# OpenDriveLab/Vista

Hardware: NVIDIA H100
Metric: denoised frames/sec at 25x576x1024, 50 EDM steps; UNet step ms (higher is better)
Workload: dtype f16 (fp32 accumulate, fp32 norms/softmax/sampler state)

## Files before the change

### vista_b200/csrc/gemm_tc.cu

```cuda
#include "gemm_tc.cuh"

namespace vb {
extern template const GemmKern* gemm_variants<32>();
extern template const GemmKern* gemm_variants<64>();
extern template const GemmKern* gemm_variants<96>();
extern template const GemmKern* gemm_variants<128>();
extern template const GemmKern* gemm_variants<160>();
extern template const GemmKern* gemm_variants<192>();
extern template const GemmKern* gemm_variants<224>();
extern template const GemmKern* gemm_variants<256>();
}

extern "C" int b200v_gemm(const b200v_gemm_desc* d, void* stream_) {
  using namespace vb;
  cudaStream_t stream = reinterpret_cast<cudaStream_t>(stream_);
  VB_REQUIRE(d && d->a && d->b && d->out, "b200v_gemm: null pointer");
  VB_REQUIRE(d->cin > 0 && d->cin % 64 == 0, "b200v_gemm: cin=%d must be a positive multiple of 64", d->cin);
  VB_REQUIRE(d->ntaps >= 1 && d->ntaps <= 9, "b200v_gemm: ntaps=%d out of range", d->ntaps);
  VB_REQUIRE(d->N > 0 && d->N % 8 == 0, "b200v_gemm: N=%d must be a multiple of 8", d->N);
  VB_REQUIRE(d->tile_n >= 32 && d->tile_n <= 256 && d->tile_n % 32 == 0, "b200v_gemm: tile_n=%d invalid", d->tile_n);
  VB_REQUIRE(d->lda % 8 == 0 && d->ldo % 8 == 0, "b200v_gemm: lda/ldo must be multiples of 8");
  VB_REQUIRE(d->act >= 0 && d->act <= 3, "b200v_gemm: act=%d invalid", d->act);
  VB_REQUIRE(!(d->act == 2 && (d->tile_n % 64 != 0 || d->N % d->tile_n != 0 || d->out_f32)),
             "b200v_gemm: GEGLU needs tile_n %% 64 == 0, N %% tile_n == 0, 16-bit output");
  VB_REQUIRE(!(d->act == 2 && (d->rowvec || d->res1 || d->res2)), "b200v_gemm: GEGLU epilogue takes bias only");
  VB_REQUIRE(!(d->act == 3 && (d->rowvec || d->res1 || d->res2 || d->bf16 || d->out_f32 || d->stats)),
             "b200v_gemm: the GELU epilogue takes bias only, fp16 operands and output (compiled variant)");
  VB_REQUIRE(!d->res1 || d->ld_res1 % 8 == 0, "b200v_gemm: ld_res1 must be a multiple of 8");
  VB_REQUIRE(!d->res2 || d->ld_res2 % 8 == 0, "b200v_gemm: ld_res2 must be a multiple of 8");
  VB_REQUIRE(!d->rowvec || (d->ld_rowvec % 4 == 0 && d->rv_div > 0 && d->rv_mod > 0), "b200v_gemm: bad rowvec args");
  VB_REQUIRE((reinterpret_cast<uintptr_t>(d->a) & 15) == 0 && (reinterpret_cast<uintptr_t>(d->b) & 15) == 0 &&
                 (reinterpret_cast<uintptr_t>(d->out) & 15) == 0,
             "b200v_gemm: a/b/out must be 16-byte aligned");

  TGParams p;
  memset(&p, 0, sizeof(p));
  p.a_mode = d->a_mode;
  p.tokens = d->tokens;
  const long long K = (long long)d->ntaps * d->cin;
  CUtensorMap tmA, tmB;
  if (d->a_mode == 0) {
    VB_REQUIRE(d->ntaps == 1 && d->h_pad == 0, "b200v_gemm: linear mode takes one tap and no halo rows");
    VB_REQUIRE(d->tokens > 0 && d->tokens < (1ll << 31) - 256, "b200v_gemm: tokens out of range");
    p.W = (int)d->tokens; p.H = 1; p.NB = 1;
    p.BW = 128; p.BH = 1; p.BB = 1;
    p.tiles_w = (int)((d->tokens + 127) / 128); p.tiles_h = 1;
    p.m_tiles = p.tiles_w;
    uint64_t dims[2] = {(uint64_t)d->cin, (uint64_t)d->tokens};
    uint64_t strides[1] = {(uint64_t)d->lda * 2};
    uint32_t box[2] = {64, 128};
    uint32_t es[2] = {1, 1};
    if (encode_tmap_16bit(&tmA, d->a, 2, dims, strides, box, es, d->bf16)) return 3;
  } else {
    VB_REQUIRE(d->a_mode == 1 || d->a_mode == 2, "b200v_gemm: a_mode=%d invalid", d->a_mode);
    const long long out_tokens = d->a_mode == 2 ? 4ll * d->tokens : d->tokens;
    VB_REQUIRE(d->W > 0 && d->H > 0 && d->NB > 0 && (long long)d->W * d->H * d->NB == d->tokens &&
                   out_tokens < (1ll << 31) - 256,
               "b200v_gemm: W*H*NB != tokens (or output tokens >= 2^31)");
    VB_REQUIRE(d->a_mode == 1 || (d->h_pad == 0 && d->act == 0 && !d->rowvec && !d->res1 && !d->res2 && !d->bf16 &&
                                  !d->out_f32 && d->s_acc == 1.0f),
               "b200v_gemm: the upsampling mode (a_mode 2) takes bias and fused statistics only, fp16 in and out");
    VB_REQUIRE(d->box_w > 0 && d->box_h > 0 && d->box_b > 0 && d->box_w * d->box_h * d->box_b == 128,
               "b200v_gemm: box_w*box_h*box_b must be 128");
    p.W = d->W; p.H = d->H; p.NB = d->NB;
    p.BW = d->box_w; p.BH = d->box_h; p.BB = d->box_b;
    p.tiles_w = (d->W + p.BW - 1) / p.BW;
    p.tiles_h = (d->H + p.BH - 1) / p.BH;
    const int tiles_b = (d->NB + p.BB - 1) / p.BB;
    p.m_tiles = p.tiles_w * p.tiles_h * tiles_b * (d->a_mode == 2 ? 4 : 1);
    VB_REQUIRE(d->h_pad >= 0 && d->h_pad <= 4, "b200v_gemm: h_pad=%d out of range", d->h_pad);
    const uint64_t He = (uint64_t)d->H + 2ull * d->h_pad;
    uint64_t dims[4] = {(uint64_t)d->cin, (uint64_t)d->W, He, (uint64_t)d->NB};
    uint64_t strides[3] = {(uint64_t)d->lda * 2, (uint64_t)d->lda * 2 * d->W, (uint64_t)d->lda * 2 * d->W * He};
    uint32_t box[4] = {64, (uint32_t)p.BW, (uint32_t)p.BH, (uint32_t)p.BB};
    uint32_t es[4] = {1, 1, 1, 1};
    if (encode_tmap_16bit(&tmA, d->a, 4, dims, strides, box, es, d->bf16)) return 3;
  }
  {
    uint64_t dims[2] = {(uint64_t)K, (uint64_t)d->N};
    uint64_t strides[1] = {(uint64_t)K * 2};
    uint32_t box[2] = {64, (uint32_t)d->tile_n};
    uint32_t es[2] = {1, 1};
    if (encode_tmap_16bit(&tmB, d->b, 2, dims, strides, box, es, d->bf16)) return 3;
  }
  p.ntaps = d->ntaps;
  p.kc_per_tap = d->cin / 64;
  for (int i = 0; i < 9; ++i) {
    p.dh[i] = d->dh[i] + (d->a_mode == 1 ? d->h_pad : 0);
    p.dw[i] = d->dw[i];
  }
  p.N = d->N;
  p.n_tiles = (d->N + d->tile_n - 1) / d->tile_n;
  p.stage_bytes = kABytes + ((d->tile_n * 128 + 1023) / 1024) * 1024;
  constexpr int kMaxSmem = 227 * 1024;
  p.nstages = (kMaxSmem - 2048 - kStagingBytes) / p.stage_bytes;
  if (p.nstages > kMaxStages) p.nstages = kMaxStages;
  const long long kMaxLd = (1ll << 31) - 1;
  VB_REQUIRE(d->ldo * (d->out_f32 ? 4 : 2) <= kMaxLd && d->ld_rowvec * 4 <= kMaxLd && d->ld_res1 * 2 <= kMaxLd &&
                 d->ld_res2 * 2 <= kMaxLd,
             "b200v_gemm: row stride too large");
  for (p.bw_sh = 0; (1 << p.bw_sh) < p.BW; ++p.bw_sh) {}
  for (p.bh_sh = 0; (1 << p.bh_sh) < p.BH; ++p.bh_sh) {}
  p.out = d->out; p.ldo_b = (int)(d->ldo * (d->out_f32 ? 4 : 2)); p.out_f32 = d->out_f32; p.act = d->act;
  p.bias = d->bias;
  p.rowvec = d->rowvec; p.ld_rowvec_b = (int)(d->ld_rowvec * 4); p.rv_div = d->rv_div > 0 ? d->rv_div : 1;
  p.rv_mod = d->rv_mod > 0 ? d->rv_mod : 1;
  p.res1 = d->res1; p.ld_res1_b = (int)(d->ld_res1 * 2); p.s_res1 = d->s_res1;
  p.res2 = d->res2; p.ld_res2_b = (int)(d->ld_res2 * 2); p.s_res2 = d->s_res2;
  p.s_acc = d->s_acc;
  VB_REQUIRE(!(d->res2 && !d->res1), "b200v_gemm: res2 without res1");
  p.stats = d->stats; p.stats_ld = (int)d->stats_ld; p.stats_col0 = d->stats_col0;
  if (d->stats) {
    VB_REQUIRE(!d->bf16 && !d->out_f32 && d->act == 0 && !d->res2 && !(d->rowvec && d->res1),
               "b200v_gemm: fused statistics need fp16 output, act 0, <= 1 residual and no rowvec + residual");
    VB_REQUIRE(d->stats_ld >= d->stats_col0 + d->N && d->stats_col0 % 4 == 0 && d->stats_ld % 4 == 0 &&
                   (reinterpret_cast<uintptr_t>(d->stats) & 15) == 0,
               "b200v_gemm: bad stats_ld / stats_col0 / alignment");
    VB_REQUIRE(d->a_mode == 0 || (p.BB == 1 && d->W % p.BW == 0 && d->H % p.BH == 0 &&
                                  (d->a_mode == 2 || p.BW == d->W || p.BH == 1)),
               "b200v_gemm: fused statistics need token tiles of 128 consecutive tokens, or boxes that tile each frame "
               "in upsampling mode (box %d x %d x %d on %d x %d)",
               p.BW, p.BH, p.BB, d->W, d->H);
  }

  const int smem_bytes = 1024 + 1024 + p.nstages * p.stage_bytes + kStagingBytes;
  int variant = d->bf16 ? 12 : 7;
  if (d->stats) {
    variant = 9 + (d->rowvec ? 2 : (d->res1 ? 1 : 0));
  } else if (!d->bf16 && !d->out_f32) {
    const int nres = (d->res1 ? 1 : 0) + (d->res2 ? 1 : 0);
    if (d->act == 0 && !d->rowvec) variant = nres;
    else if (d->act == 0 && nres <= 1) variant = 3 + nres;
    else if (d->act == 1 && !d->rowvec && nres == 0) variant = 5;
    else if (d->act == 2) variant = 6;
    else if (d->act == 3) variant = 8;
  }
  static const GemmKern* const kByWidth[8] = {gemm_variants<32>(),  gemm_variants<64>(),  gemm_variants<96>(),
                                              gemm_variants<128>(), gemm_variants<160>(), gemm_variants<192>(),
                                              gemm_variants<224>(), gemm_variants<256>()};
  static bool attr_set[64] = {false};
  if (vb::first_use_on_device(attr_set)) {
    for (int w = 0; w < 8; ++w)
      for (int i = 0; i < kGemmVariants; ++i)
        VB_CHECK_CUDA(cudaFuncSetAttribute(kByWidth[w][i], cudaFuncAttributeMaxDynamicSharedMemorySize, kMaxSmem));
  }
  const long long total = (long long)p.m_tiles * p.n_tiles;
  int grid = device_sm_count();
  if (total < grid) grid = (int)total;
  const GemmKern k = kByWidth[d->tile_n / 32 - 1][variant];
  k<<<grid, kGemmThreads, smem_bytes, stream>>>(tmA, tmB, p);
  VB_CHECK_CUDA(cudaGetLastError());
  return 0;
}
```

### vista_b200/csrc/gemm_tc.cuh

```cuda
#pragma once
#include "../../include/vista_b200.h"
#include "host.cuh"
#include "ptx.cuh"

namespace vb {

constexpr int kMaxStages = 8;
constexpr int kABytes = 128 * 64 * 2;
constexpr int kStageBufBytes = 64 * 32 * 4;
constexpr int kStagingBytes = 2 * 2 * kStageBufBytes;
constexpr int kGemmThreads = 384;

struct TGParams {
  int a_mode;
  int W, H, NB;
  int BW, BH, BB;
  int bw_sh, bh_sh;
  int tiles_w, tiles_h;
  int m_tiles, n_tiles;
  int ntaps, kc_per_tap;
  int dh[9], dw[9];
  int N;
  int nstages, stage_bytes;
  long long tokens;
  void* out;
  int ldo_b;
  int out_f32, act;
  const float* bias;
  const float* rowvec;
  int ld_rowvec_b;
  int rv_div, rv_mod;
  const void* res1;
  int ld_res1_b;
  float s_res1;
  const void* res2;
  int ld_res2_b;
  float s_res2;
  float s_acc;
  float* stats;
  int stats_ld, stats_col0;
};

__device__ __forceinline__ float2 unpack2(uint32_t w, int bf16) {
  if (bf16) return make_float2(__uint_as_float(w << 16), __uint_as_float(w & 0xFFFF0000u));
  return __half22float2(*reinterpret_cast<const __half2*>(&w));
}
__device__ __forceinline__ uint32_t pack2(float a, float b, int bf16) {
  if (bf16) {
    __nv_bfloat162 t = __floats2bfloat162_rn(a, b);
    return *reinterpret_cast<uint32_t*>(&t);
  }
  __half2 t = __floats2half2_rn(a, b);
  return *reinterpret_cast<uint32_t*>(&t);
}

template <int TN, bool BF16>
__device__ __forceinline__ void issue_kchunk(float (&acc)[TN / 2], uint64_t adesc, uint64_t bdesc, bool overwrite) {
#pragma unroll
  for (int kk = 0; kk < 4; ++kk)
    wgmma_ss<TN, BF16>(acc, adesc + (uint64_t)(2 * kk), bdesc + (uint64_t)(2 * kk), (overwrite && kk == 0) ? 0 : 1);
}

template <int TN, int ACT_, bool RV_, int NRES_, bool GEN, bool STATS = false, bool BF16 = false>
__global__ void __launch_bounds__(kGemmThreads, 1)
tapgemm_kernel(const __grid_constant__ CUtensorMap tmA, const __grid_constant__ CUtensorMap tmB, const TGParams p) {
  extern __shared__ uint8_t smem_raw[];
  const uint32_t raw = smem_u32(smem_raw);
  uint8_t* smem = smem_raw + (((raw + 1023u) & ~1023u) - raw);
  uint64_t* full = reinterpret_cast<uint64_t*>(smem);
  uint64_t* empty = full + kMaxStages;
  uint8_t* stages = smem + 1024;

  const int warp = threadIdx.x >> 5, lane = threadIdx.x & 31;
  const int KC = p.ntaps * p.kc_per_tap;
  const int total_tiles = p.m_tiles * p.n_tiles;

  if (threadIdx.x == 0) {
    for (int i = 0; i < p.nstages; ++i) {
      mbar_init(&full[i], 1);
      mbar_init(&empty[i], 8);
    }
    fence_barrier_init();
  }
  if (warp == 8 && lane == 0) {
    tma_prefetch_desc(&tmA);
    tma_prefetch_desc(&tmB);
  }
  __syncthreads();

  if (warp >= 8) {
    setmaxnreg_dec<40>();
    if (warp == 8 && lane == 0) {
      int stage = 0;
      uint32_t phase = 0;
      const uint32_t tx = (uint32_t)(kABytes + TN * 128);
      for (int tile = blockIdx.x; tile < total_tiles; tile += gridDim.x) {
        const int m_blk = tile / p.n_tiles, n_blk = tile - m_blk * p.n_tiles;
        const int up = p.a_mode == 2;
        const int box = up ? (m_blk >> 2) : m_blk;
        const int px = up ? (m_blk & 1) : 0, py = up ? ((m_blk >> 1) & 1) : 0;
        const int tw = box % p.tiles_w;
        const int th = (box / p.tiles_w) % p.tiles_h;
        const int tb = box / (p.tiles_w * p.tiles_h);
        const int w0 = tw * p.BW, h0 = th * p.BH, b0 = tb * p.BB;
        const int n0 = n_blk * TN;
        for (int kc = 0; kc < KC; ++kc) {
          mbar_wait_relaxed(&empty[stage], phase ^ 1, 1);
          uint8_t* sA = stages + stage * p.stage_bytes;
          uint8_t* sB = sA + kABytes;
          const int tap = kc / p.kc_per_tap;
          const int c0 = (kc - tap * p.kc_per_tap) * 64;
          mbar_expect_tx(&full[stage], tx);
          const int dw = up ? ((px + p.dw[tap]) >> 1) : p.dw[tap];
          const int dh = up ? ((py + p.dh[tap]) >> 1) : p.dh[tap];
          if (p.a_mode == 0)
            tma_load_2d(sA, &tmA, &full[stage], c0, w0);
          else
            tma_load_4d(sA, &tmA, &full[stage], c0, w0 + dw, h0 + dh, b0);
          tma_load_2d(sB, &tmB, &full[stage], kc * 64, n0);
          if (++stage == p.nstages) {
            stage = 0;
            phase ^= 1;
          }
        }
      }
    }
    return;
  }

  setmaxnreg_inc<232>();
  const int wg = warp >> 2, wq = warp & 3;
  const int act = GEN ? p.act : ACT_;
  const bool has_rv = GEN ? (p.rowvec != nullptr) : RV_;
  const bool has_r1 = GEN ? (p.res1 != nullptr) : (NRES_ >= 1);
  const bool has_r2 = GEN ? (p.res2 != nullptr) : (NRES_ >= 2);
  constexpr bool bf16 = BF16;
  const bool f32o = GEN ? (p.out_f32 != 0) : false;
  const bool has_bias = p.bias != nullptr;
  constexpr int half = TN >> 1;
  const int tile_out_cols = (act == 2) ? half : TN;
  const int n_out_total = (act == 2) ? (p.N >> 1) : p.N;
  const int G = tile_out_cols >> 5;
  const int out_es = f32o ? 4 : 2;
  const char* r1p = reinterpret_cast<const char*>(p.res1);
  const char* r2p = reinterpret_cast<const char*>(p.res2);
  const uint64_t desc0 = make_desc_sw128(smem_u32(stages), 16, 1024);
  const uint32_t stage_step = (uint32_t)p.stage_bytes >> 4;
  const uint32_t stg0 = smem_u32(stages + p.nstages * p.stage_bytes) + wg * 2 * kStageBufBytes;
  const int g = lane >> 2, c = lane & 3;
  const int rh = wq & 1, chh = wq >> 1;
  const int ch = lane & 3, rsub = lane >> 2;
  int stage = 0;
  uint32_t phase = 0;
  uint32_t gcount = 0;

  float acc[TN / 2];
  for (int tile = blockIdx.x; tile < total_tiles; tile += gridDim.x) {
    const int m_blk = tile / p.n_tiles, n_blk = tile - m_blk * p.n_tiles;
    int prev = -1;
    for (int kc = 0; kc < KC; ++kc) {
      mbar_wait(&full[stage], phase, 3);
      const uint64_t ad = desc0 + (uint64_t)(stage * stage_step + wg * 512);
      const uint64_t bd = desc0 + (uint64_t)(stage * stage_step + (kABytes >> 4));
      wgmma_fence();
      issue_kchunk<TN, BF16>(acc, ad, bd, kc == 0);
      wgmma_commit();
      if (prev >= 0) {
        wgmma_wait<1>();
        if (lane == 0) mbar_arrive(&empty[prev]);
      }
      prev = stage;
      if (++stage == p.nstages) {
        stage = 0;
        phase ^= 1;
      }
    }
    wgmma_wait<0>();
    if (lane == 0) mbar_arrive(&empty[prev]);
    fence_regs(acc);

    const int r_own = wg * 64 + rh * 32 + lane;
    int token_own, valid_own;
    if (p.a_mode == 0) {
      token_own = m_blk * 128 + r_own;
      valid_own = token_own < p.tokens;
    } else {
      const int up = p.a_mode == 2;
      const int box = up ? (m_blk >> 2) : m_blk;
      const int tw = box % p.tiles_w;
      const int t2 = box / p.tiles_w;
      const int th = t2 % p.tiles_h;
      const int tb = t2 / p.tiles_h;
      const int ww = r_own & (p.BW - 1), hh = (r_own >> p.bw_sh) & (p.BH - 1), bb = r_own >> (p.bw_sh + p.bh_sh);
      const int w = tw * p.BW + ww, h = th * p.BH + hh, b = tb * p.BB + bb;
      valid_own = (w < p.W) && (h < p.H) && (b < p.NB);
      token_own = up ? ((2 * (b * p.H + h) + ((m_blk >> 1) & 1)) * 2 * p.W + 2 * w + (m_blk & 1))
                     : (b * p.H + h) * p.W + w;
    }
    if (!valid_own) token_own = 0;
    const uint32_t vrows = __ballot_sync(0xffffffffu, valid_own) >> rsub;
    int tok[4], rvrow[4];
    {
      const int rv_own = has_rv ? (token_own / p.rv_div) % p.rv_mod : 0;
#pragma unroll
      for (int i = 0; i < 4; ++i) {
        tok[i] = __shfl_sync(0xffffffffu, token_own, i * 8 + rsub);
        rvrow[i] = has_rv ? __shfl_sync(0xffffffffu, rv_own, i * 8 + rsub) : 0;
      }
    }
    const int n_out_base = n_blk * tile_out_cols;
#pragma unroll
    for (int k = 0; k < TN / 32; ++k) {
      if (k >= G) break;
      const int c0 = k * 32;
      if (n_out_base + c0 >= n_out_total) break;
      const uint32_t stg = stg0 + (gcount & 1) * kStageBufBytes;
      ++gcount;
      float f[16];
#pragma unroll
      for (int j = 0; j < 16; ++j) f[j] = acc[16 * k + j];
      if (act == 2) {
        float gt[16];
        const int kg = (half >> 5) + k;
#pragma unroll
        for (int j = 0; j < 16; ++j) gt[j] = 0.f;
#pragma unroll
        for (int q = 0; q < TN / 32; ++q)
          if (q == kg) {
#pragma unroll
            for (int j = 0; j < 16; ++j) gt[j] = acc[16 * q + j];
          }
        const int nb = n_blk * TN + c0;
#pragma unroll
        for (int ii = 0; ii < 4; ++ii) {
          float2 bv = make_float2(0.f, 0.f), bg = make_float2(0.f, 0.f);
          if (has_bias) {
            bv = __ldg(reinterpret_cast<const float2*>(p.bias + nb + 8 * ii + 2 * c));
            bg = __ldg(reinterpret_cast<const float2*>(p.bias + nb + half + 8 * ii + 2 * c));
          }
          f[4 * ii + 0] = geglu_fast(f[4 * ii + 0] + bv.x, gt[4 * ii + 0] + bg.x);
          f[4 * ii + 1] = geglu_fast(f[4 * ii + 1] + bv.y, gt[4 * ii + 1] + bg.y);
          f[4 * ii + 2] = geglu_fast(f[4 * ii + 2] + bv.x, gt[4 * ii + 2] + bg.x);
          f[4 * ii + 3] = geglu_fast(f[4 * ii + 3] + bv.y, gt[4 * ii + 3] + bg.y);
        }
      }
#pragma unroll
      for (int ii = 0; ii < 4; ++ii) {
        const int chunk = 2 * ii + (c >> 1), sub = (c & 1) * 8;
#pragma unroll
        for (int hr = 0; hr < 2; ++hr) {
          const int row = wq * 16 + g + 8 * hr;
          asm volatile("st.shared.v2.f32 [%0], {%1, %2};" ::"r"(stg + row * 128 + ((chunk ^ (row & 7)) << 4) + sub),
                       "f"(f[4 * ii + 2 * hr]), "f"(f[4 * ii + 2 * hr + 1])
                       : "memory");
        }
      }
      asm volatile("bar.sync %0, 128;" ::"r"(1 + wg) : "memory");
      {
        const int n = n_out_base + c0 + chh * 16 + ch * 4;
        const bool n_ok = n + 4 <= n_out_total;
        float4 bs = make_float4(0.f, 0.f, 0.f, 0.f);
        float sa = 1.0f;
        if (act != 2) {
          sa = p.s_acc;
          if (has_bias && n_ok) {
            const float4 b4 = __ldg(reinterpret_cast<const float4*>(p.bias + n));
            bs = make_float4(b4.x * sa, b4.y * sa, b4.z * sa, b4.w * sa);
          }
        }
        char* obase = reinterpret_cast<char*>(p.out) + (long long)n * out_es;
        const char* r1base = r1p + (long long)n * 2;
        const char* r2base = r2p + (long long)n * 2;
        const char* rvbase = reinterpret_cast<const char*>(p.rowvec) + (long long)n * 4;
        float cs[4] = {0.f, 0.f, 0.f, 0.f}, cq[4] = {0.f, 0.f, 0.f, 0.f};
        float4 v[4], rv[4];
        uint2 u1[4], u2[4];
#pragma unroll
        for (int i = 0; i < 4; ++i) {
          const int row = rh * 32 + i * 8 + rsub;
          const int chunk = chh * 4 + ch;
          asm volatile("ld.shared.v4.f32 {%0, %1, %2, %3}, [%4];"
                       : "=f"(v[i].x), "=f"(v[i].y), "=f"(v[i].z), "=f"(v[i].w)
                       : "r"(stg + row * 128 + ((chunk ^ (row & 7)) << 4)));
          const bool ok = n_ok && ((vrows >> (8 * i)) & 1u);
          rv[i] = make_float4(0.f, 0.f, 0.f, 0.f);
          u1[i] = make_uint2(0, 0);
          u2[i] = make_uint2(0, 0);
          if (has_rv && ok) rv[i] = __ldg(reinterpret_cast<const float4*>(rvbase + (long long)rvrow[i] * p.ld_rowvec_b));
          if (has_r1 && ok) u1[i] = __ldg(reinterpret_cast<const uint2*>(r1base + (long long)tok[i] * p.ld_res1_b));
          if (has_r2 && ok) u2[i] = __ldg(reinterpret_cast<const uint2*>(r2base + (long long)tok[i] * p.ld_res2_b));
        }
#pragma unroll
        for (int i = 0; i < 4; ++i) {
          const bool ok = n_ok && ((vrows >> (8 * i)) & 1u);
          float4 o = v[i];
          if (act != 2) {
            o.x = fmaf(o.x, sa, bs.x); o.y = fmaf(o.y, sa, bs.y); o.z = fmaf(o.z, sa, bs.z); o.w = fmaf(o.w, sa, bs.w);
            if (has_rv) { o.x += rv[i].x; o.y += rv[i].y; o.z += rv[i].z; o.w += rv[i].w; }
            if (act == 1) { o.x = silu_f(o.x); o.y = silu_f(o.y); o.z = silu_f(o.z); o.w = silu_f(o.w); }
            if (!GEN && act == 3) { o.x = gelu_erf_fast(o.x); o.y = gelu_erf_fast(o.y); o.z = gelu_erf_fast(o.z); o.w = gelu_erf_fast(o.w); }
            if (has_r1) {
              const float2 a = unpack2(u1[i].x, bf16), b = unpack2(u1[i].y, bf16);
              o.x = fmaf(p.s_res1, a.x, o.x); o.y = fmaf(p.s_res1, a.y, o.y);
              o.z = fmaf(p.s_res1, b.x, o.z); o.w = fmaf(p.s_res1, b.y, o.w);
            }
            if (has_r2) {
              const float2 a = unpack2(u2[i].x, bf16), b = unpack2(u2[i].y, bf16);
              o.x = fmaf(p.s_res2, a.x, o.x); o.y = fmaf(p.s_res2, a.y, o.y);
              o.z = fmaf(p.s_res2, b.x, o.z); o.w = fmaf(p.s_res2, b.y, o.w);
            }
          }
          if (STATS && ok) {
            cs[0] += o.x; cs[1] += o.y; cs[2] += o.z; cs[3] += o.w;
            cq[0] = fmaf(o.x, o.x, cq[0]); cq[1] = fmaf(o.y, o.y, cq[1]);
            cq[2] = fmaf(o.z, o.z, cq[2]); cq[3] = fmaf(o.w, o.w, cq[3]);
          }
          char* optr = obase + (long long)tok[i] * p.ldo_b;
          if (f32o) {
            if (ok) *reinterpret_cast<float4*>(optr) = o;
          } else {
            const uint2 pk = make_uint2(pack2(o.x, o.y, bf16), pack2(o.z, o.w, bf16));
            if (ok) *reinterpret_cast<uint2*>(optr) = pk;
          }
        }
        if (STATS) {
#pragma unroll
          for (int off = 4; off < 32; off <<= 1) {
#pragma unroll
            for (int q = 0; q < 4; ++q) {
              cs[q] += __shfl_xor_sync(0xffffffffu, cs[q], off);
              cq[q] += __shfl_xor_sync(0xffffffffu, cq[q], off);
            }
          }
          if (rsub == 0 && n_ok) {
            float* dst = p.stats + (((long long)m_blk * 4 + wg * 2 + rh) * p.stats_ld + p.stats_col0 + n) * 2;
            *reinterpret_cast<float4*>(dst) = make_float4(cs[0], cq[0], cs[1], cq[1]);
            *reinterpret_cast<float4*>(dst + 4) = make_float4(cs[2], cq[2], cs[3], cq[3]);
          }
        }
      }
    }
  }
}

using GemmKern = void (*)(const CUtensorMap, const CUtensorMap, const TGParams);
constexpr int kGemmVariants = 13;

template <int TN>
const GemmKern* gemm_variants() {
  static const GemmKern v[kGemmVariants] = {
      tapgemm_kernel<TN, 0, false, 0, false>,       tapgemm_kernel<TN, 0, false, 1, false>,
      tapgemm_kernel<TN, 0, false, 2, false>,       tapgemm_kernel<TN, 0, true, 0, false>,
      tapgemm_kernel<TN, 0, true, 1, false>,        tapgemm_kernel<TN, 1, false, 0, false>,
      tapgemm_kernel<TN, 2, false, 0, false>,       tapgemm_kernel<TN, 0, true, 2, true>,
      tapgemm_kernel<TN, 3, false, 0, false>,       tapgemm_kernel<TN, 0, false, 0, false, true>,
      tapgemm_kernel<TN, 0, false, 1, false, true>, tapgemm_kernel<TN, 0, true, 0, false, true>,
      tapgemm_kernel<TN, 0, true, 2, true, false, true>};
  return v;
}

}
```

### vista_b200/csrc/ptx.cuh

```cuda
#pragma once
#include <cuda.h>
#include <cuda_bf16.h>
#include <cuda_fp16.h>
#include <cuda_runtime.h>
#include <stdint.h>
#include <stdio.h>

namespace vb {

__device__ __forceinline__ uint32_t smem_u32(const void* p) {
  return static_cast<uint32_t>(__cvta_generic_to_shared(p));
}

__device__ __forceinline__ void mbar_init(uint64_t* bar, uint32_t count) {
  asm volatile("mbarrier.init.shared::cta.b64 [%0], %1;" ::"r"(smem_u32(bar)), "r"(count) : "memory");
}
__device__ __forceinline__ void fence_barrier_init() {
  asm volatile("fence.mbarrier_init.release.cluster;" ::: "memory");
}
__device__ __forceinline__ void mbar_expect_tx(uint64_t* bar, uint32_t bytes) {
  asm volatile("mbarrier.arrive.expect_tx.shared::cta.b64 _, [%0], %1;" ::"r"(smem_u32(bar)), "r"(bytes) : "memory");
}
__device__ __forceinline__ void mbar_arrive(uint64_t* bar) {
  asm volatile("mbarrier.arrive.shared::cta.b64 _, [%0];" ::"r"(smem_u32(bar)) : "memory");
}
__device__ __forceinline__ bool mbar_try_wait(uint64_t* bar, uint32_t parity) {
  uint32_t ok;
  asm volatile(
      "{\n\t.reg .pred p;\n\t"
      "mbarrier.try_wait.parity.shared::cta.b64 p, [%1], %2;\n\t"
      "selp.u32 %0, 1, 0, p;\n\t}"
      : "=r"(ok)
      : "r"(smem_u32(bar)), "r"(parity)
      : "memory");
  return ok != 0;
}
__device__ __forceinline__ bool mbar_test_wait(uint64_t* bar, uint32_t parity) {
  uint32_t ok;
  asm volatile(
      "{\n\t.reg .pred p;\n\t"
      "mbarrier.test_wait.parity.shared::cta.b64 p, [%1], %2;\n\t"
      "selp.u32 %0, 1, 0, p;\n\t}"
      : "=r"(ok)
      : "r"(smem_u32(bar)), "r"(parity)
      : "memory");
  return ok != 0;
}
#ifndef VB_WAIT_TIMEOUT_CYCLES
#define VB_WAIT_TIMEOUT_CYCLES (4000000000ll)
#endif
__device__ __forceinline__ void mbar_wait(uint64_t* bar, uint32_t parity, int tag = 0) {
  (void)tag;
  if (mbar_try_wait(bar, parity)) return;
  long long t0 = 0;
  for (uint32_t spins = 1;; ++spins) {
    if (mbar_try_wait(bar, parity)) return;
    if ((spins & 4095u) == 0u) {
      const long long now = clock64();
      if (t0 == 0) t0 = now;
      if (now - t0 > VB_WAIT_TIMEOUT_CYCLES) __trap();
    }
  }
}
__device__ __forceinline__ void mbar_wait_relaxed(uint64_t* bar, uint32_t parity, int tag = 0) {
  (void)tag;
  for (int i = 0; i < 4; ++i)
    if (mbar_try_wait(bar, parity)) return;
  long long t0 = 0;
  for (uint32_t spins = 1;; ++spins) {
    __nanosleep(32);
    if (mbar_try_wait(bar, parity)) return;
    if ((spins & 4095u) == 0u) {
      const long long now = clock64();
      if (t0 == 0) t0 = now;
      if (now - t0 > VB_WAIT_TIMEOUT_CYCLES) __trap();
    }
  }
}

__device__ __forceinline__ void fence_proxy_async_smem() {
  asm volatile("fence.proxy.async.shared::cta;" ::: "memory");
}

__device__ __forceinline__ void tma_prefetch_desc(const CUtensorMap* m) {
  asm volatile("prefetch.tensormap [%0];" ::"l"(reinterpret_cast<uint64_t>(m)) : "memory");
}
__device__ __forceinline__ void tma_load_2d(void* dst, const CUtensorMap* m, uint64_t* bar, int c0, int c1) {
  asm volatile(
      "cp.async.bulk.tensor.2d.shared::cluster.global.tile.mbarrier::complete_tx::bytes [%0], [%1, {%3, %4}], [%2];"
      ::"r"(smem_u32(dst)), "l"(reinterpret_cast<uint64_t>(m)), "r"(smem_u32(bar)), "r"(c0), "r"(c1)
      : "memory");
}
__device__ __forceinline__ void tma_load_3d(void* dst, const CUtensorMap* m, uint64_t* bar, int c0, int c1, int c2) {
  asm volatile(
      "cp.async.bulk.tensor.3d.shared::cluster.global.tile.mbarrier::complete_tx::bytes [%0], [%1, {%3, %4, %5}], [%2];"
      ::"r"(smem_u32(dst)), "l"(reinterpret_cast<uint64_t>(m)), "r"(smem_u32(bar)), "r"(c0), "r"(c1), "r"(c2)
      : "memory");
}
__device__ __forceinline__ void tma_load_4d(void* dst, const CUtensorMap* m, uint64_t* bar, int c0, int c1, int c2,
                                            int c3) {
  asm volatile(
      "cp.async.bulk.tensor.4d.shared::cluster.global.tile.mbarrier::complete_tx::bytes [%0], [%1, {%3, %4, %5, %6}], [%2];"
      ::"r"(smem_u32(dst)), "l"(reinterpret_cast<uint64_t>(m)), "r"(smem_u32(bar)), "r"(c0), "r"(c1), "r"(c2), "r"(c3)
      : "memory");
}

__device__ __forceinline__ uint64_t make_desc_sw128(uint32_t smem_addr, uint32_t lbo_bytes, uint32_t sbo_bytes) {
  uint64_t d = 0;
  d |= static_cast<uint64_t>((smem_addr & 0x3FFFFu) >> 4);
  d |= static_cast<uint64_t>((lbo_bytes >> 4) & 0x3FFFu) << 16;
  d |= static_cast<uint64_t>((sbo_bytes >> 4) & 0x3FFFu) << 32;
  d |= static_cast<uint64_t>(1) << 62;
  return d;
}
__device__ __forceinline__ void wgmma_fence() { asm volatile("wgmma.fence.sync.aligned;" ::: "memory"); }
__device__ __forceinline__ void wgmma_commit() { asm volatile("wgmma.commit_group.sync.aligned;" ::: "memory"); }
template <int N>
__device__ __forceinline__ void wgmma_wait() { asm volatile("wgmma.wait_group.sync.aligned %0;" ::"n"(N) : "memory"); }
template <int R>
__device__ __forceinline__ void setmaxnreg_inc() { asm volatile("setmaxnreg.inc.sync.aligned.u32 %0;" ::"n"(R)); }
template <int R>
__device__ __forceinline__ void setmaxnreg_dec() { asm volatile("setmaxnreg.dec.sync.aligned.u32 %0;" ::"n"(R)); }
template <int N>
__device__ __forceinline__ void fence_regs(float (&r)[N]) {
#pragma unroll
  for (int i = 0; i < N; ++i) asm volatile("" : "+f"(r[i])::"memory");
}

#define VB_R16_0 "%3, %4, %5, %6, %7, %8, %9, %10, %11, %12, %13, %14, %15, %16, %17, %18"
#define VB_R16_1 ", %19, %20, %21, %22, %23, %24, %25, %26, %27, %28, %29, %30, %31, %32, %33, %34"
#define VB_R16_2 ", %35, %36, %37, %38, %39, %40, %41, %42, %43, %44, %45, %46, %47, %48, %49, %50"
#define VB_R16_3 ", %51, %52, %53, %54, %55, %56, %57, %58, %59, %60, %61, %62, %63, %64, %65, %66"
#define VB_R16_4 ", %67, %68, %69, %70, %71, %72, %73, %74, %75, %76, %77, %78, %79, %80, %81, %82"
#define VB_R16_5 ", %83, %84, %85, %86, %87, %88, %89, %90, %91, %92, %93, %94, %95, %96, %97, %98"
#define VB_R16_6 ", %99, %100, %101, %102, %103, %104, %105, %106, %107, %108, %109, %110, %111, %112, %113, %114"
#define VB_R16_7 ", %115, %116, %117, %118, %119, %120, %121, %122, %123, %124, %125, %126, %127, %128, %129, %130"
#define VB_D16(b)                                                                                                      \
  "+f"(d[b + 0]), "+f"(d[b + 1]), "+f"(d[b + 2]), "+f"(d[b + 3]), "+f"(d[b + 4]), "+f"(d[b + 5]), "+f"(d[b + 6]),      \
      "+f"(d[b + 7]), "+f"(d[b + 8]), "+f"(d[b + 9]), "+f"(d[b + 10]), "+f"(d[b + 11]), "+f"(d[b + 12]),               \
      "+f"(d[b + 13]), "+f"(d[b + 14]), "+f"(d[b + 15])
#define VB_WGMMA_SS(N, T, REGS, ...)                                                                                   \
  asm volatile("{\n\t.reg .pred p;\n\tsetp.ne.b32 p, %2, 0;\n\t"                                                      \
               "wgmma.mma_async.sync.aligned.m64n" #N "k16.f32." T "." T " {" REGS "}, %0, %1, p, 1, 1, 0, 0;\n\t}" \
               : "+l"(da), "+l"(db), "+r"(scale_d), __VA_ARGS__)
#define VB_WGMMA_SS_T(N, REGS, ...)                                                                                    \
  do {                                                                                                                 \
    if constexpr (BF16) VB_WGMMA_SS(N, "bf16", REGS, __VA_ARGS__);                                                     \
    else VB_WGMMA_SS(N, "f16", REGS, __VA_ARGS__);                                                                     \
  } while (0)
template <int N, bool BF16>
__device__ __forceinline__ void wgmma_ss(float (&d)[N / 2], uint64_t da, uint64_t db, int scale_d) {
  static_assert(N >= 32 && N <= 256 && N % 32 == 0, "wgmma_ss: N must be a multiple of 32 in [32, 256]");
  if constexpr (N == 32) VB_WGMMA_SS_T(32, VB_R16_0, VB_D16(0));
  else if constexpr (N == 64) VB_WGMMA_SS_T(64, VB_R16_0 VB_R16_1, VB_D16(0), VB_D16(16));
  else if constexpr (N == 96) VB_WGMMA_SS_T(96, VB_R16_0 VB_R16_1 VB_R16_2, VB_D16(0), VB_D16(16), VB_D16(32));
  else if constexpr (N == 128)
    VB_WGMMA_SS_T(128, VB_R16_0 VB_R16_1 VB_R16_2 VB_R16_3, VB_D16(0), VB_D16(16), VB_D16(32), VB_D16(48));
  else if constexpr (N == 160)
    VB_WGMMA_SS_T(160, VB_R16_0 VB_R16_1 VB_R16_2 VB_R16_3 VB_R16_4, VB_D16(0), VB_D16(16), VB_D16(32), VB_D16(48),
                  VB_D16(64));
  else if constexpr (N == 192)
    VB_WGMMA_SS_T(192, VB_R16_0 VB_R16_1 VB_R16_2 VB_R16_3 VB_R16_4 VB_R16_5, VB_D16(0), VB_D16(16), VB_D16(32),
                  VB_D16(48), VB_D16(64), VB_D16(80));
  else if constexpr (N == 224)
    VB_WGMMA_SS_T(224, VB_R16_0 VB_R16_1 VB_R16_2 VB_R16_3 VB_R16_4 VB_R16_5 VB_R16_6, VB_D16(0), VB_D16(16),
                  VB_D16(32), VB_D16(48), VB_D16(64), VB_D16(80), VB_D16(96));
  else
    VB_WGMMA_SS_T(256, VB_R16_0 VB_R16_1 VB_R16_2 VB_R16_3 VB_R16_4 VB_R16_5 VB_R16_6 VB_R16_7, VB_D16(0), VB_D16(16),
                  VB_D16(32), VB_D16(48), VB_D16(64), VB_D16(80), VB_D16(96), VB_D16(112));
}
#undef VB_WGMMA_SS_T
#undef VB_WGMMA_SS
#undef VB_D16
#undef VB_R16_0
#undef VB_R16_1
#undef VB_R16_2
#undef VB_R16_3
#undef VB_R16_4
#undef VB_R16_5
#undef VB_R16_6
#undef VB_R16_7

__device__ __forceinline__ void wgmma_m64n128_f16(float (&d)[64], uint64_t da, uint64_t db, int scale_d) {
  asm volatile(
      "{\n\t.reg .pred p;\n\tsetp.ne.b32 p, %66, 0;\n\t"
      "wgmma.mma_async.sync.aligned.m64n128k16.f32.f16.f16 "
      "{%0, %1, %2, %3, %4, %5, %6, %7, %8, %9, %10, %11, %12, %13, %14, %15, %16, %17, %18, %19, %20, %21, %22, %23, %24, %25, %26, %27, %28, %29, %30, %31, %32, %33, %34, %35, %36, %37, %38, %39, %40, %41, %42, %43, %44, %45, %46, %47, %48, %49, %50, %51, %52, %53, %54, %55, %56, %57, %58, %59, %60, %61, %62, %63}, "
      "%64, %65, p, 1, 1, 0, 0;\n\t}"
      : "+f"(d[0]), "+f"(d[1]), "+f"(d[2]), "+f"(d[3]), "+f"(d[4]), "+f"(d[5]), "+f"(d[6]), "+f"(d[7]), "+f"(d[8]), "+f"(d[9]), "+f"(d[10]), "+f"(d[11]), "+f"(d[12]), "+f"(d[13]), "+f"(d[14]), "+f"(d[15]), "+f"(d[16]), "+f"(d[17]), "+f"(d[18]), "+f"(d[19]), "+f"(d[20]), "+f"(d[21]), "+f"(d[22]), "+f"(d[23]), "+f"(d[24]), "+f"(d[25]), "+f"(d[26]), "+f"(d[27]), "+f"(d[28]), "+f"(d[29]), "+f"(d[30]), "+f"(d[31]), "+f"(d[32]), "+f"(d[33]), "+f"(d[34]), "+f"(d[35]), "+f"(d[36]), "+f"(d[37]), "+f"(d[38]), "+f"(d[39]), "+f"(d[40]), "+f"(d[41]), "+f"(d[42]), "+f"(d[43]), "+f"(d[44]), "+f"(d[45]), "+f"(d[46]), "+f"(d[47]), "+f"(d[48]), "+f"(d[49]), "+f"(d[50]), "+f"(d[51]), "+f"(d[52]), "+f"(d[53]), "+f"(d[54]), "+f"(d[55]), "+f"(d[56]), "+f"(d[57]), "+f"(d[58]), "+f"(d[59]), "+f"(d[60]), "+f"(d[61]), "+f"(d[62]), "+f"(d[63])
      : "l"(da), "l"(db), "r"(scale_d));
}

__device__ __forceinline__ void wgmma_m64n64_f16_rs_tb(float (&d)[32], const uint32_t (&a)[4], uint64_t db, int scale_d) {
  asm volatile(
      "{\n\t.reg .pred p;\n\tsetp.ne.b32 p, %37, 0;\n\t"
      "wgmma.mma_async.sync.aligned.m64n64k16.f32.f16.f16 "
      "{%0, %1, %2, %3, %4, %5, %6, %7, %8, %9, %10, %11, %12, %13, %14, %15, %16, %17, %18, %19, %20, %21, %22, %23, %24, %25, %26, %27, %28, %29, %30, %31}, "
      "{%32, %33, %34, %35}, %36, p, 1, 1, 1;\n\t}"
      : "+f"(d[0]), "+f"(d[1]), "+f"(d[2]), "+f"(d[3]), "+f"(d[4]), "+f"(d[5]), "+f"(d[6]), "+f"(d[7]), "+f"(d[8]), "+f"(d[9]), "+f"(d[10]), "+f"(d[11]), "+f"(d[12]), "+f"(d[13]), "+f"(d[14]), "+f"(d[15]), "+f"(d[16]), "+f"(d[17]), "+f"(d[18]), "+f"(d[19]), "+f"(d[20]), "+f"(d[21]), "+f"(d[22]), "+f"(d[23]), "+f"(d[24]), "+f"(d[25]), "+f"(d[26]), "+f"(d[27]), "+f"(d[28]), "+f"(d[29]), "+f"(d[30]), "+f"(d[31])
      : "r"(a[0]), "r"(a[1]), "r"(a[2]), "r"(a[3]), "l"(db), "r"(scale_d));
}

__device__ __forceinline__ float silu_f(float x) {
  float e, r;
  asm("ex2.approx.ftz.f32 %0, %1;" : "=f"(e) : "f"(x * -1.4426950408889634f));
  asm("rcp.approx.ftz.f32 %0, %1;" : "=f"(r) : "f"(1.0f + e));
  return x * r;
}
__device__ __forceinline__ float gelu_erf_f(float x) { return 0.5f * x * (1.0f + erff(x * 0.70710678118654752f)); }
__device__ __forceinline__ float gelu_erf_fast(float x) {
  const float ax = fabsf(x) * 0.70710678118654752f;
  float t;
  asm("rcp.approx.ftz.f32 %0, %1;" : "=f"(t) : "f"(fmaf(0.3275911f, ax, 1.0f)));
  float poly = fmaf(t, 1.061405429f, -1.453152027f);
  poly = fmaf(t, poly, 1.421413741f);
  poly = fmaf(t, poly, -0.284496736f);
  poly = fmaf(t, poly, 0.254829592f);
  float e;
  asm("ex2.approx.ftz.f32 %0, %1;" : "=f"(e) : "f"(ax * (ax * -1.4426950408889634f)));
  const float r = (0.5f * x) * ((poly * t) * e);
  return x < 0.0f ? r : x - r;
}
__device__ __forceinline__ float geglu_fast(float v, float x) {
  float t;
  asm("rcp.approx.ftz.f32 %0, %1;" : "=f"(t) : "f"(fmaf(fabsf(x), 0.23164190f, 1.0f)));
  float poly = fmaf(t, 0.5307027145f, -0.7265760135f);
  poly = fmaf(t, poly, 0.7107068705f);
  poly = fmaf(t, poly, -0.142248368f);
  poly = fmaf(t, poly, 0.127414796f);
  float e;
  asm("ex2.approx.ftz.f32 %0, %1;" : "=f"(e) : "f"((x * -0.72134752044f) * x));
  const float w = (poly * t) * e;
  const float vx = v * x;
  const float r = vx * w;
  return x < 0.0f ? r : vx - r;
}
__device__ __forceinline__ float ex2_f(float x) {
  float y;
  asm("ex2.approx.ftz.f32 %0, %1;" : "=f"(y) : "f"(x));
  return y;
}

}
```

Baseline: 1.290.

## Launch GEMM as 2-CTA clusters sharing weight tiles via TMA multicast

```diff
diff --git a/vista_b200/csrc/gemm_tc.cu b/vista_b200/csrc/gemm_tc.cu
--- a/vista_b200/csrc/gemm_tc.cu
+++ b/vista_b200/csrc/gemm_tc.cu
@@ -9,6 +9,31 @@
 extern template const GemmKern* gemm_variants<192>();
 extern template const GemmKern* gemm_variants<224>();
 extern template const GemmKern* gemm_variants<256>();
+
+constexpr int kMaxSmem = 227 * 1024;
+
+static int gemm_smem_bytes(int tn, int* stage_bytes, int* nstages) {
+  *stage_bytes = kABytes + ((tn * 128 + 1023) / 1024) * 1024;
+  *nstages = (kMaxSmem - 2048 - kStagingBytes) / *stage_bytes;
+  if (*nstages > kMaxStages) *nstages = kMaxStages;
+  return 1024 + 1024 + *nstages * *stage_bytes + kStagingBytes;
+}
+
+static cudaLaunchConfig_t gemm_launch_config(int grid, int smem_bytes, cudaStream_t stream, cudaLaunchAttribute* attr) {
+  cudaLaunchConfig_t cfg;
+  memset(&cfg, 0, sizeof(cfg));
+  cfg.gridDim = dim3(grid, 1, 1);
+  cfg.blockDim = dim3(kGemmThreads, 1, 1);
+  cfg.dynamicSmemBytes = smem_bytes;
+  cfg.stream = stream;
+  attr->id = cudaLaunchAttributeClusterDimension;
+  attr->val.clusterDim.x = 2;
+  attr->val.clusterDim.y = 1;
+  attr->val.clusterDim.z = 1;
+  cfg.attrs = attr;
+  cfg.numAttrs = 1;
+  return cfg;
+}
 }
 
 extern "C" int b200v_gemm(const b200v_gemm_desc* d, void* stream_) {
@@ -79,7 +104,7 @@
   {
     uint64_t dims[2] = {(uint64_t)K, (uint64_t)d->N};
     uint64_t strides[1] = {(uint64_t)K * 2};
-    uint32_t box[2] = {64, (uint32_t)d->tile_n};
+    uint32_t box[2] = {64, (uint32_t)d->tile_n / 2};
     uint32_t es[2] = {1, 1};
     if (encode_tmap_16bit(&tmB, d->b, 2, dims, strides, box, es, d->bf16)) return 3;
   }
@@ -91,10 +116,8 @@
   }
   p.N = d->N;
   p.n_tiles = (d->N + d->tile_n - 1) / d->tile_n;
-  p.stage_bytes = kABytes + ((d->tile_n * 128 + 1023) / 1024) * 1024;
-  constexpr int kMaxSmem = 227 * 1024;
-  p.nstages = (kMaxSmem - 2048 - kStagingBytes) / p.stage_bytes;
-  if (p.nstages > kMaxStages) p.nstages = kMaxStages;
+  p.pairs = (p.m_tiles + 1) / 2 * p.n_tiles;
+  const int smem_bytes = gemm_smem_bytes(d->tile_n, &p.stage_bytes, &p.nstages);
   const long long kMaxLd = (1ll << 31) - 1;
   VB_REQUIRE(d->ldo * (d->out_f32 ? 4 : 2) <= kMaxLd && d->ld_rowvec * 4 <= kMaxLd && d->ld_res1 * 2 <= kMaxLd &&
                  d->ld_res2 * 2 <= kMaxLd,
@@ -123,7 +146,6 @@
                p.BW, p.BH, p.BB, d->W, d->H);
   }
 
-  const int smem_bytes = 1024 + 1024 + p.nstages * p.stage_bytes + kStagingBytes;
   int variant = d->bf16 ? 12 : 7;
   if (d->stats) {
     variant = 9 + (d->rowvec ? 2 : (d->res1 ? 1 : 0));
@@ -139,16 +161,26 @@
                                               gemm_variants<128>(), gemm_variants<160>(), gemm_variants<192>(),
                                               gemm_variants<224>(), gemm_variants<256>()};
   static bool attr_set[64] = {false};
+  static int max_clusters[64][8];
+  int dev = 0;
+  VB_CHECK_CUDA(cudaGetDevice(&dev));
+  VB_REQUIRE(dev >= 0 && dev < 64, "b200v_gemm: device %d out of range", dev);
   if (vb::first_use_on_device(attr_set)) {
-    for (int w = 0; w < 8; ++w)
+    for (int w = 0; w < 8; ++w) {
       for (int i = 0; i < kGemmVariants; ++i)
         VB_CHECK_CUDA(cudaFuncSetAttribute(kByWidth[w][i], cudaFuncAttributeMaxDynamicSharedMemorySize, kMaxSmem));
+      int sb, ns;
+      cudaLaunchAttribute attr;
+      const cudaLaunchConfig_t cfg = gemm_launch_config(2, gemm_smem_bytes(32 * (w + 1), &sb, &ns), stream, &attr);
+      VB_CHECK_CUDA(cudaOccupancyMaxActiveClusters(&max_clusters[dev][w], (const void*)kByWidth[w][0], &cfg));
+      VB_REQUIRE(max_clusters[dev][w] > 0, "b200v_gemm: no 2-CTA cluster of tile width %d fits on the device",
+                 32 * (w + 1));
+    }
   }
-  const long long total = (long long)p.m_tiles * p.n_tiles;
-  int grid = device_sm_count();
-  if (total < grid) grid = (int)total;
+  const int clusters = p.pairs < max_clusters[dev][d->tile_n / 32 - 1] ? p.pairs : max_clusters[dev][d->tile_n / 32 - 1];
   const GemmKern k = kByWidth[d->tile_n / 32 - 1][variant];
-  k<<<grid, kGemmThreads, smem_bytes, stream>>>(tmA, tmB, p);
-  VB_CHECK_CUDA(cudaGetLastError());
+  cudaLaunchAttribute attr;
+  const cudaLaunchConfig_t cfg = gemm_launch_config(2 * clusters, smem_bytes, stream, &attr);
+  VB_CHECK_CUDA(cudaLaunchKernelEx(&cfg, k, tmA, tmB, p));
   return 0;
 }
diff --git a/vista_b200/csrc/gemm_tc.cuh b/vista_b200/csrc/gemm_tc.cuh
--- a/vista_b200/csrc/gemm_tc.cuh
+++ b/vista_b200/csrc/gemm_tc.cuh
@@ -18,6 +18,7 @@
   int bw_sh, bh_sh;
   int tiles_w, tiles_h;
   int m_tiles, n_tiles;
+  int pairs;
   int ntaps, kc_per_tap;
   int dh[9], dw[9];
   int N;
@@ -73,12 +74,12 @@
 
   const int warp = threadIdx.x >> 5, lane = threadIdx.x & 31;
   const int KC = p.ntaps * p.kc_per_tap;
-  const int total_tiles = p.m_tiles * p.n_tiles;
+  const uint32_t rank = cluster_ctarank();
 
   if (threadIdx.x == 0) {
     for (int i = 0; i < p.nstages; ++i) {
       mbar_init(&full[i], 1);
-      mbar_init(&empty[i], 8);
+      mbar_init(&empty[i], 16);
     }
     fence_barrier_init();
   }
@@ -86,16 +87,19 @@
     tma_prefetch_desc(&tmA);
     tma_prefetch_desc(&tmB);
   }
-  __syncthreads();
+  cluster_sync();
 
   if (warp >= 8) {
     setmaxnreg_dec<40>();
     if (warp == 8 && lane == 0) {
       int stage = 0;
       uint32_t phase = 0;
-      const uint32_t tx = (uint32_t)(kABytes + TN * 128);
-      for (int tile = blockIdx.x; tile < total_tiles; tile += gridDim.x) {
-        const int m_blk = tile / p.n_tiles, n_blk = tile - m_blk * p.n_tiles;
+      constexpr int kBHalfRows = TN / 2;
+      for (int pp = blockIdx.x >> 1; pp < p.pairs; pp += gridDim.x >> 1) {
+        const int n_blk = pp % p.n_tiles;
+        const int m_blk = 2 * (pp / p.n_tiles) + (int)rank;
+        const bool active = m_blk < p.m_tiles;
+        const uint32_t tx = (uint32_t)((active ? kABytes : 0) + TN * 128);
         const int up = p.a_mode == 2;
         const int box = up ? (m_blk >> 2) : m_blk;
         const int px = up ? (m_blk & 1) : 0, py = up ? ((m_blk >> 1) & 1) : 0;
@@ -113,15 +117,25 @@
           mbar_expect_tx(&full[stage], tx);
           const int dw = up ? ((px + p.dw[tap]) >> 1) : p.dw[tap];
           const int dh = up ? ((py + p.dh[tap]) >> 1) : p.dh[tap];
-          if (p.a_mode == 0)
-            tma_load_2d(sA, &tmA, &full[stage], c0, w0);
-          else
-            tma_load_4d(sA, &tmA, &full[stage], c0, w0 + dw, h0 + dh, b0);
-          tma_load_2d(sB, &tmB, &full[stage], kc * 64, n0);
+          if (active) {
+            if (p.a_mode == 0)
+              tma_load_2d(sA, &tmA, &full[stage], c0, w0);
+            else
+              tma_load_4d(sA, &tmA, &full[stage], c0, w0 + dw, h0 + dh, b0);
+          }
+          tma_load_2d_multicast(sB + rank * kBHalfRows * 128, &tmB, &full[stage], kc * 64, n0 + (int)rank * kBHalfRows,
+                                0x3);
           if (++stage == p.nstages) {
             stage = 0;
             phase ^= 1;
           }
+        }
+      }
+      for (int i = 0; i < p.nstages; ++i) {
+        mbar_wait_relaxed(&empty[stage], phase ^ 1, 2);
+        if (++stage == p.nstages) {
+          stage = 0;
+          phase ^= 1;
         }
       }
     }
@@ -153,10 +167,29 @@
   int stage = 0;
   uint32_t phase = 0;
   uint32_t gcount = 0;
+  const uint32_t peer_empty0 = mapa_shared(smem_u32(empty), rank ^ 1u);
+  auto release = [&](int s) {
+    if (lane == 0) {
+      mbar_arrive(&empty[s]);
+      mbar_arrive_cluster(peer_empty0 + 8u * (uint32_t)s);
+    }
+  };
 
   float acc[TN / 2];
-  for (int tile = blockIdx.x; tile < total_tiles; tile += gridDim.x) {
-    const int m_blk = tile / p.n_tiles, n_blk = tile - m_blk * p.n_tiles;
+  for (int pp = blockIdx.x >> 1; pp < p.pairs; pp += gridDim.x >> 1) {
+    const int n_blk = pp % p.n_tiles;
+    const int m_blk = 2 * (pp / p.n_tiles) + (int)rank;
+    if (m_blk >= p.m_tiles) {
+      for (int kc = 0; kc < KC; ++kc) {
+        mbar_wait(&full[stage], phase, 3);
+        release(stage);
+        if (++stage == p.nstages) {
+          stage = 0;
+          phase ^= 1;
+        }
+      }
+      continue;
+    }
     int prev = -1;
     for (int kc = 0; kc < KC; ++kc) {
       mbar_wait(&full[stage], phase, 3);
@@ -167,7 +200,7 @@
       wgmma_commit();
       if (prev >= 0) {
         wgmma_wait<1>();
-        if (lane == 0) mbar_arrive(&empty[prev]);
+        release(prev);
       }
       prev = stage;
       if (++stage == p.nstages) {
@@ -176,7 +209,7 @@
       }
     }
     wgmma_wait<0>();
-    if (lane == 0) mbar_arrive(&empty[prev]);
+    release(prev);
     fence_regs(acc);
 
     const int r_own = wg * 64 + rh * 32 + lane;
@@ -209,6 +242,25 @@
       }
     }
     const int n_out_base = n_blk * tile_out_cols;
+    uint2 u1[4], u2[4];
+    float4 rv[4];
+    auto load_row_operands = [&](int kg) {
+      const int n = n_out_base + kg * 32 + chh * 16 + ch * 4;
+      const bool n_ok = n + 4 <= n_out_total;
+#pragma unroll
+      for (int i = 0; i < 4; ++i) {
+        const bool ok = n_ok && ((vrows >> (8 * i)) & 1u);
+        u1[i] = make_uint2(0, 0);
+        u2[i] = make_uint2(0, 0);
+        rv[i] = make_float4(0.f, 0.f, 0.f, 0.f);
+        if (has_rv && ok)
+          rv[i] = __ldg(reinterpret_cast<const float4*>(reinterpret_cast<const char*>(p.rowvec) + (long long)n * 4 +
+                                                        (long long)rvrow[i] * p.ld_rowvec_b));
+        if (has_r1 && ok) u1[i] = __ldg(reinterpret_cast<const uint2*>(r1p + (long long)n * 2 + (long long)tok[i] * p.ld_res1_b));
+        if (has_r2 && ok) u2[i] = __ldg(reinterpret_cast<const uint2*>(r2p + (long long)n * 2 + (long long)tok[i] * p.ld_res2_b));
+      }
+    };
+    load_row_operands(0);
 #pragma unroll
     for (int k = 0; k < TN / 32; ++k) {
       if (k >= G) break;
@@ -269,12 +321,8 @@
           }
         }
         char* obase = reinterpret_cast<char*>(p.out) + (long long)n * out_es;
-        const char* r1base = r1p + (long long)n * 2;
-        const char* r2base = r2p + (long long)n * 2;
-        const char* rvbase = reinterpret_cast<const char*>(p.rowvec) + (long long)n * 4;
         float cs[4] = {0.f, 0.f, 0.f, 0.f}, cq[4] = {0.f, 0.f, 0.f, 0.f};
-        float4 v[4], rv[4];
-        uint2 u1[4], u2[4];
+        float4 v[4];
 #pragma unroll
         for (int i = 0; i < 4; ++i) {
           const int row = rh * 32 + i * 8 + rsub;
@@ -283,12 +331,6 @@
                        : "=f"(v[i].x), "=f"(v[i].y), "=f"(v[i].z), "=f"(v[i].w)
                        : "r"(stg + row * 128 + ((chunk ^ (row & 7)) << 4)));
           const bool ok = n_ok && ((vrows >> (8 * i)) & 1u);
-          rv[i] = make_float4(0.f, 0.f, 0.f, 0.f);
-          u1[i] = make_uint2(0, 0);
-          u2[i] = make_uint2(0, 0);
-          if (has_rv && ok) rv[i] = __ldg(reinterpret_cast<const float4*>(rvbase + (long long)rvrow[i] * p.ld_rowvec_b));
-          if (has_r1 && ok) u1[i] = __ldg(reinterpret_cast<const uint2*>(r1base + (long long)tok[i] * p.ld_res1_b));
-          if (has_r2 && ok) u2[i] = __ldg(reinterpret_cast<const uint2*>(r2base + (long long)tok[i] * p.ld_res2_b));
         }
 #pragma unroll
         for (int i = 0; i < 4; ++i) {
@@ -323,6 +365,7 @@
             if (ok) *reinterpret_cast<uint2*>(optr) = pk;
           }
         }
+        if (k + 1 < TN / 32) load_row_operands(k + 1);
         if (STATS) {
 #pragma unroll
           for (int off = 4; off < 32; off <<= 1) {
diff --git a/vista_b200/csrc/ptx.cuh b/vista_b200/csrc/ptx.cuh
--- a/vista_b200/csrc/ptx.cuh
+++ b/vista_b200/csrc/ptx.cuh
@@ -82,6 +82,23 @@
   asm volatile("fence.proxy.async.shared::cta;" ::: "memory");
 }
 
+__device__ __forceinline__ uint32_t cluster_ctarank() {
+  uint32_t r;
+  asm volatile("mov.u32 %0, %%cluster_ctarank;" : "=r"(r));
+  return r;
+}
+__device__ __forceinline__ uint32_t mapa_shared(uint32_t addr, uint32_t rank) {
+  uint32_t r;
+  asm volatile("mapa.shared::cluster.u32 %0, %1, %2;" : "=r"(r) : "r"(addr), "r"(rank));
+  return r;
+}
+__device__ __forceinline__ void mbar_arrive_cluster(uint32_t cluster_addr) {
+  asm volatile("mbarrier.arrive.shared::cluster.b64 _, [%0];" ::"r"(cluster_addr) : "memory");
+}
+__device__ __forceinline__ void cluster_sync() {
+  asm volatile("barrier.cluster.arrive.release;\n\tbarrier.cluster.wait.acquire;" ::: "memory");
+}
+
 __device__ __forceinline__ void tma_prefetch_desc(const CUtensorMap* m) {
   asm volatile("prefetch.tensormap [%0];" ::"l"(reinterpret_cast<uint64_t>(m)) : "memory");
 }
@@ -89,6 +106,14 @@
   asm volatile(
       "cp.async.bulk.tensor.2d.shared::cluster.global.tile.mbarrier::complete_tx::bytes [%0], [%1, {%3, %4}], [%2];"
       ::"r"(smem_u32(dst)), "l"(reinterpret_cast<uint64_t>(m)), "r"(smem_u32(bar)), "r"(c0), "r"(c1)
+      : "memory");
+}
+__device__ __forceinline__ void tma_load_2d_multicast(void* dst, const CUtensorMap* m, uint64_t* bar, int c0, int c1,
+                                                      uint16_t cta_mask) {
+  asm volatile(
+      "cp.async.bulk.tensor.2d.shared::cluster.global.tile.mbarrier::complete_tx::bytes.multicast::cluster"
+      " [%0], [%1, {%3, %4}], [%2], %5;"
+      ::"r"(smem_u32(dst)), "l"(reinterpret_cast<uint64_t>(m)), "r"(smem_u32(bar)), "r"(c0), "r"(c1), "h"(cta_mask)
       : "memory");
 }
 __device__ __forceinline__ void tma_load_3d(void* dst, const CUtensorMap* m, uint64_t* bar, int c0, int c1, int c2) {
```

Measured after the change: 1.328 (median of 6 runs). 2.9% higher.
